# wenet-e2e/wenet

Measured on AMD Instinct MI355X. Metric: audio-seconds/sec (RTF^-1), 12L Conformer fbank80, ctc_prefix_beam_search, higher is better.
Workload: dtype f32 (feed-forward and subsampling-conv2 GEMMs: fp32 operands as three exact bf16 planes, six plane products on the bf16 matrix cores, f32 accumulate -- error <= the v_mfma_f32 kernel's, tests/test_gpu_x6.py; everything else v_mfma_f32)

## Files before the change

include/wenet_amd.h:

```cpp
#ifndef WENET_AMD_H_
#define WENET_AMD_H_

#include <stdint.h>

#ifdef __cplusplus
extern "C" {
#endif

typedef struct wn_model wn_model;

typedef struct {
  int32_t feat_dim;
  int32_t d_model;
  int32_t n_heads;
  int32_t ffn_dim;
  int32_t n_layers;
  int32_t cnn_kernel;
  int32_t causal;
  int32_t use_dynamic_chunk;
  int32_t static_chunk_size;
  int32_t vocab;
  int32_t has_cmvn;
  int32_t dec_heads;
  int32_t dec_ffn_dim;
// ... 193 lines not shown
int wn_op_mx_quantize(const float* x_dev, int32_t rows, int32_t K, void* q_dev,
                      void* scale_dev, void* stream);
int wn_op_ffn_fused(const float* X_dev, const float* W1_dev, const float* b1_dev,
                    const float* W2_dev, const float* b2_dev, float* x_inout_dev,
                    const float* ln_w_dev, const float* ln_b_dev, float* y_out_dev,
                    int32_t M, int32_t D, int32_t F, int32_t act, float alpha, float eps,
                    void* stream);
int wn_op_gemm_x6(const float* A_dev, const float* W_dev, const float* bias_dev,
                  const float* resid_dev, float* C_dev, int32_t M, int32_t N, int32_t K,
                  float alpha, int32_t act, int32_t bm, int32_t reps, void* stream);
int wn_op_ffn_x6(const float* X_dev, const float* W1_dev, const float* b1_dev,
                 const float* W2_dev, const float* b2_dev, float* x_inout_dev,
                 const float* ln_w_dev, const float* ln_b_dev, float* y_out_dev, int32_t M,
                 int32_t D, int32_t F, int32_t act, float alpha, float eps, int32_t reps,
                 void* stream);
int wn_op_gemm_x6r(const float* A_dev, const float* W_dev, const float* bias_dev,
                   float* x_inout_dev, const float* ln_w_dev, const float* ln_b_dev,
                   float* y_dev, float* C_dev, int32_t M, int32_t N, int32_t epi, float alpha,
                   float eps, int32_t reps, void* stream);

int wn_op_gemm_x6r512(const float* A, const float* W, const float* bias, float* x_inout,
                      const float* ln_w, const float* ln_b, float* y, const float* W2,
                      const float* bias2, float* C, int32_t M, int32_t N, int32_t epi, float alpha,
                      float eps, int32_t reps, void* stream);
int wn_op_log_add(const double* a_dev, const double* b_dev, double* out_dev,
                  int32_t n, void* stream);
int wn_op_layernorm(const float* x_dev, const float* w_dev, const float* b_dev,
                    float* y_dev, int32_t M, int32_t D, float eps, void* stream);

typedef struct wn_attention_op {
// ... 196 lines not shown
```

wenet_amd/_lib.py:

```python
import ctypes
import os
from ctypes import (POINTER, Structure, c_char_p, c_double, c_float, c_int32,
                    c_int64, c_void_p)

_HERE = os.path.dirname(os.path.abspath(__file__))
LIB_PATH = os.path.join(_HERE, 'libwenet_amd.so')


class WnConfig(Structure):
    _fields_ = [(n, c_int32) for n in (
        'feat_dim', 'd_model', 'n_heads', 'ffn_dim', 'n_layers', 'cnn_kernel',
        'causal', 'use_dynamic_chunk', 'static_chunk_size', 'vocab',
        'has_cmvn', 'dec_heads', 'dec_ffn_dim', 'dec_layers', 'dec_r_layers',
        'bidirectional', 'sos', 'eos', 'max_pos')] + [('norm_eps', c_float)] + [
            (n, c_int32) for n in ('encoder_type', 'input_layer', 'activation',
                                   'key_bias', 'cnn_norm',
                                   'dec_activation', 'dec_key_bias', 'dec_src_key_bias',
                                   'dec_learned_pos', 'dec_max_pos')]


class WnTransducerConfig(Structure):
    _fields_ = [(n, c_int32) for n in ('pred_embed', 'pred_hidden', 'pred_layers', 'pred_out',
                                       'join_dim', 'blank')]

# ... 25 lines not shown
                ('P', c_void_p), ('ldp', c_int32), ('p_rows', c_int32),
                ('p_off', POINTER(c_int32)), ('bias_u', c_void_p), ('bias_v', c_void_p),
                ('O', c_void_p), ('ldo', c_int32),
                ('q_off', POINTER(c_int32)), ('q_len', POINTER(c_int32)),
                ('kv_off', POINTER(c_int32)), ('kv_len', POINTER(c_int32)),
                ('n_seq', c_int32), ('n_heads', c_int32), ('mask_mode', c_int32),
                ('chunk_size', c_int32), ('left_chunks', c_int32), ('scale', c_float),
                ('flags', c_int32), ('precision', c_int32), ('x6_galign', c_int32)]


EXPORTS = [
    'wn_last_error', 'wn_version', 'wn_model_create', 'wn_model_destroy', 'wn_model_clone',
    'wn_model_set_precision', 'wn_model_get_precision', 'wn_batch_size', 'wn_model_set_encode_gate', 'wn_op_gemm_bf16',
    'wn_op_gemm_bf16_stored',
    'wn_attention_beam_search', 'wn_attention_beam_search_prompt', 'wn_attention_truncated',
    'wn_op_gemm_skinny', 'wn_encode_chunk_batch', 'wn_op_gemm_lowp', 'wn_op_mx_quantize', 'wn_op_ffn_fused', 'wn_op_gemm_x6', 'wn_op_ffn_x6', 'wn_op_gemm_x6r', 'wn_op_gemm_x6r512', 'wn_profile_kernel_name', 'wn_profile_ffn_split', 'wn_profile_ffn_clocks', 'wn_profile_gemm_clocks', 'wn_filter_blank_embedding',
    'wn_workspace_create', 'wn_resample_length', 'wn_resample', 'wn_fbank', 'wn_log_mel', 'wn_encode', 'wn_encode_chunk', 'wn_set_encoder_out',
    'wn_ctc_logprobs', 'wn_set_ctc_probs', 'wn_ctc_greedy_search', 'wn_ctc_force_align',
    'wn_set_context_graph', 'wn_ctc_prefix_beam_search', 'wn_attention_rescoring', 'wn_rescore', 'wn_rescore_prefetch', 'wn_decoder_forward', 'wn_decoder_next_topk', 'wn_op_gemm',
    'wn_op_layernorm', 'wn_op_log_add', 'wn_op_attention', 'wn_op_dwconv', 'wn_op_conv1',
    'wn_op_conv2d4',
    'wn_op_ctc_rows', 'wn_debug_set', 'wn_profile_enable',
    'wn_profile_collect', 'wn_tune_set', 'wn_model_tune_set', 'wn_tune_get',
    'wn_stream_create', 'wn_stream_destroy', 'wn_stream_set_endpoint', 'wn_stream_reset',
    'wn_stream_advance', 'wn_stream_advance_encoded',
    'wn_model_create_transducer', 'wn_transducer_greedy_search', 'wn_op_lstm_step',
    'wn_op_joint_argmax', 'wn_transducer_beam_search', 'wn_op_joint_fuse_topk',
    'wn_op_rnnt_beam_step', 'wn_transducer_beam_stats',
    'wn_rnnt_stream_create', 'wn_rnnt_stream_destroy', 'wn_rnnt_stream_reset',
    'wn_rnnt_stream_advance_encoded', 'wn_rnnt_stream_state',
    'wn_transducer_score', 'wn_transducer_score_stats', 'wn_transducer_score_times',
# ... 74 lines not shown
    L.wn_attention_beam_search.argtypes = [vp, i32, i32, f32, pi32, pi32, vp]
    L.wn_attention_beam_search_prompt.argtypes = [vp, i32, i32, f32, pi32, i32, pi32, pi32, vp]
    L.wn_attention_truncated.argtypes = [vp]
    L.wn_op_gemm.argtypes = [vp, vp, vp, vp, vp, i32, i32, i32, f32, i32, vp]
    L.wn_op_gemm_skinny.argtypes = [vp, vp, vp, vp, vp, i32, i32, i32, i32, i32, i32, vp]
    L.wn_op_gemm_bf16.argtypes = L.wn_op_gemm.argtypes
    L.wn_op_gemm_bf16_stored.argtypes = [vp, vp, vp, vp, vp, i32, i32, i32, f32, i32, i32, vp]
    L.wn_op_gemm_lowp.argtypes = [vp, vp, vp, vp, vp, vp, vp, vp, i32, i32, i32, f32, i32, i32,
                                  i32, vp]
    L.wn_op_mx_quantize.argtypes = [vp, i32, i32, vp, vp, vp]
    L.wn_op_ffn_fused.argtypes = [vp, vp, vp, vp, vp, vp, vp, vp, vp, i32, i32, i32, i32, f32,
                                  f32, vp]
    L.wn_op_gemm_x6.argtypes = [vp, vp, vp, vp, vp, i32, i32, i32, f32, i32, i32, i32, vp]
    L.wn_op_ffn_x6.argtypes = [vp, vp, vp, vp, vp, vp, vp, vp, vp, i32, i32, i32, i32, f32,
                               f32, i32, vp]
    L.wn_filter_blank_embedding.argtypes = [vp, vp, pi32, pi32, vp]
    L.wn_op_gemm_x6r.argtypes = [vp, vp, vp, vp, vp, vp, vp, vp, i32, i32, i32, f32, f32, i32, vp]
    L.wn_op_gemm_x6r512.argtypes = [vp, vp, vp, vp, vp, vp, vp, vp, vp, vp, i32, i32, i32, f32, f32,
                                    i32, vp]
    L.wn_model_set_precision.argtypes = [vp, i32]
    L.wn_model_get_precision.argtypes = [vp]
    L.wn_batch_size.argtypes = [vp]
    L.wn_batch_size.restype = i32
    L.wn_model_set_encode_gate.argtypes = [vp, vp]
    L.wn_op_layernorm.argtypes = [vp, vp, vp, vp, i32, i32, f32, vp]
    L.wn_op_log_add.argtypes = [vp, vp, vp, i32, vp]
    L.wn_op_attention.argtypes = [POINTER(WnAttentionOp), pi32, vp]
    L.wn_op_dwconv.argtypes = [vp, i32, vp, vp, vp, vp, vp, i32, vp, i32, pi32, pi32, i32, i32,
                               i32, i32, i32, i32, f32, vp]
    L.wn_op_conv1.argtypes = [vp, vp, vp, vp, vp, vp, pi32, pi32, i32, i32, i32, i32, i32, i32,
# ... 87 lines not shown
```

wenet_amd/build.py:

```python
import concurrent.futures
import hashlib
import os
import shutil
import subprocess
import sys

HERE = os.path.dirname(os.path.abspath(__file__))
CSRC = os.path.join(HERE, 'csrc')
OBJ = os.path.join(HERE, '..', 'build', 'obj')
LIB = os.path.join(HERE, 'libwenet_amd.so')
SOURCES = ['gemm.hip', 'gemm_bf16.hip', 'gemm_bf16s.hip', 'gemm_bf16p.hip', 'gemm_skinny.hip', 'ffn_fused.hip', 'gemm_rowln.hip', 'gemm_x6.hip', 'ffn_x6f.hip', 'gemm_x6r.hip', 'gemm_x6r512.hip', 'attn_search.hip', 'encoder_kernels.hip', 'attention_bf16.hip', 'attention_x6.hip', 'ctc.hip', 'ctc_align.hip', 'fbank.hip',
           'logmel.hip', 'model.hip', 'conformer.hip', 'cabi_model.hip', 'cabi_encode.hip', 'cabi_ctc.hip', 'cabi_align.hip',
           'cabi_decoder.hip', 'cabi_ops.hip', 'transducer.hip', 'transducer_beam.hip',
           'cabi_transducer.hip', 'transducer_score.hip', 'cabi_transducer_score.hip',
           'transducer_stream.hip', 'cabi_transducer_stream.hip']
FLAGS = ['--offload-arch=gfx950', '-O3', '-std=c++17', '-fPIC',
         '-fno-gpu-rdc', '-Wno-unused-result']
if os.environ.get('WN_ABLATION') == '1':
    FLAGS.append('-DWN_ABLATION')
if os.environ.get('WN_EXACT') == '1':
    FLAGS.append('-DWN_EXACT_TRANSCENDENTALS')
EXTRA_FLAGS = {'ffn_x6f.hip': ['-fno-slp-vectorize'], 'gemm_x6r.hip': ['-fno-slp-vectorize'], 'gemm_x6r512.hip': ['-fno-slp-vectorize'],
               'attention_bf16.hip': ['-fno-slp-vectorize']}


def _hipcc():
    for c in (os.environ.get('HIPCC'), shutil.which('hipcc'),
              '/opt/rocm/bin/hipcc'):
        if c and os.path.exists(c):
            return c
    raise RuntimeError('hipcc not found')


def build_host_ext(force: bool = False) -> str:
    import sysconfig
    src = os.path.join(HERE, 'cext', 'nbest_lists.c')
    out = os.path.join(HERE, '_nbest_lists' + sysconfig.get_config_var('EXT_SUFFIX'))
# ... 72 lines not shown
```

wenet_amd/csrc/cabi_ops.hip:

```cpp
#include "model_state.h"
#include "x6.h"

namespace wn {
namespace {

__global__ __launch_bounds__(256) void conv1_image_unpack_kernel(
    const char* __restrict__ img, int tiles, const int* __restrict__ t1_off,
    const int* __restrict__ t1_len, int F1, int C, float* __restrict__ out) {
  const int b = blockIdx.y;
  const int n = t1_len[b] * F1 * (C / 8);
  const int ne = (F1 + 1) / 2;
  for (int i = blockIdx.x * 256 + threadIdx.x; i < n; i += gridDim.x * 256) {
    const int cg = i % (C / 8), px = i / (C / 8);
    const int fr = px / F1, pos = px - fr * F1;
    const int f1 = pos < ne ? 2 * pos : 2 * (pos - ne) + 1;
    const int row = (t1_off[b] + fr) * F1;
    const char* src = img + x3_piece(cg >> 1, tiles, row + pos, cg & 1);
    const bf16x8 p0 = *reinterpret_cast<const bf16x8*>(src);
    const bf16x8 p1 = *reinterpret_cast<const bf16x8*>(src + X3_REC);
    const bf16x8 p2 = *reinterpret_cast<const bf16x8*>(src + 2 * X3_REC);
    float* o = out + ((int64_t)row + f1) * C + cg * 8;
#pragma unroll
    for (int e = 0; e < 8; ++e) o[e] = ((float)p0[e] + (float)p1[e]) + (float)p2[e];
  }
// ... 169 lines not shown
  if (tune().x6_af32 != 0 && (int64_t)M * K * 4 < ((int64_t)1 << 31)) {
    a.A = A; a.lda = K; a.a_bytes = (int64_t)M * K * 4;
  } else {
    WN_TRY(a3.ensure(x6_bytes(M, K)));
    WN_TRY(x6_split(A, M, K, K, a3.as<char>(), s));
    a.A3 = a3.as<char>();
  }
  a.B3 = w3.as<char>(); a.M = M; a.N = N; a.K = K; a.bm = bm;
  if (bm == 120) { a.bm = 128; a.nw = 8; }
  if (bm == 129) { a.bm = 128; a.nw = 4; }
  a.bias = bias; a.resid = resid; a.ldr = N; a.alpha = alpha; a.act = act; a.C = C; a.ldc = N;
  for (int r = 0; r < (reps > 0 ? reps : 1); ++r) WN_TRY(gemm_x6(a, s));
  return 0;
}

int wn_op_ffn_x6(const float* X, const float* W1, const float* b1, const float* W2,
                 const float* b2, float* x, const float* ln_w, const float* ln_b, float* y,
                 int32_t M, int32_t D, int32_t F, int32_t act, float alpha, float eps,
                 int32_t reps, void* stream) {
  WN_CHECK(X && W1 && b1 && W2 && b2 && x && ln_w && ln_b && y, "ffn_x6: null argument");
  WN_CHECK(M > 0 && (D == 256 || D == 512) && F > 0 && F % 64 == 0, "ffn_x6: shape");
  hipStream_t s = (hipStream_t)stream;
  static thread_local DevBuf x3, w13, w23, h3, part;
  if (tune().ffn_x6f != 0 && tune().x6_af32 == 0 && ffn_x6f_supported(M, D, F, act)) {
    FfnX6Args a;
    a.S = ffn_x6f_split(M, F);
    WN_TRY(w13.ensure(x6_bytes(F, D)));
    WN_TRY(w23.ensure(x6_bytes(D, F)));
    WN_TRY(part.ensure((size_t)a.S * M * D * sizeof(float)));
    WN_TRY(x6_split(W1, F, D, D, w13.as<char>(), s));
    WN_TRY(x6_split_perm(W2, D, F, F, w23.as<char>(), s));
    a.X = X; a.ldx = D; a.W13 = w13.as<char>(); a.W2p = w23.as<char>(); a.b1 = b1;
    a.P = part.as<float>(); a.M = M; a.D = D; a.F = F; a.act = act;
    if (tune().ffn_ximg == 2) {
      WN_TRY(x3.ensure(x6_bytes(M, D)));
      WN_TRY(x6_split(X, M, D, D, x3.as<char>(), s));
      a.X3 = x3.as<char>(); a.X = nullptr;
    }
    for (int r = 0; r < (reps > 0 ? reps : 1); ++r) WN_TRY(ffn_x6f(a, s));
    return ffn_reduce_ln(x, part.as<float>(), a.S, b2, alpha, ln_w, ln_b, nullptr, nullptr, y, M,
                         D, eps, 0, s);
  }
  const int S = ffn_x6_split(M, F);
  WN_TRY(x3.ensure(x6_bytes(M, D)));
  WN_TRY(w13.ensure(x6_bytes(F, D)));
  WN_TRY(w23.ensure(x6_bytes(D, F)));
// ... 488 lines not shown
```

wenet_amd/csrc/conformer.hip:

```cpp
#include <algorithm>
#include "model_state.h"

namespace {
struct ProfBracket {
  wn_model* m;
  hipStream_t s;
  bool on = false;
  int record(int which) { WN_HIP(hipEventRecord(m->prof_ev[m->prof_used + which], s)); return 0; }
  int begin() {
    on = m->prof_on && (m->prof_seq++ % m->prof_stride) == 0;
    if (!on) return 0;
    if (m->prof_used + 2 > m->prof_ev.size())
      for (int i = 0; i < 64; ++i) {
        hipEvent_t e;
        WN_HIP(hipEventCreate(&e));
        m->prof_ev.push_back(e);
      }
    return record(0);
  }
  int end(double flops, const char* kernel) {
    if (!on) return 0;
    WN_TRY(record(1));
    m->prof_used += 2;
    m->prof_flops += flops;
// ... 97 lines not shown
  const int d = m->cfg.d_model, M = m->rows, F = w1.out;
  const bool ximg = m->t1_img_ok;
  m->t1_img_ok = false;
  const int route = ffn_x6_route(m, w1, w2, act);
  WN_CHECK(route != 0 || !ximg,
           "ffn_x6_try: LN(x) was left as a plane image but no six-product form takes it");
  if (route == 0) return 0;
  auto i1 = W.x6_at.find(w1.w), i2 = W.x6_at.find(w2.w);
  ProfBracket pb{m, s};
  if (route == 1) {
    FfnX6Args a;
    a.S = ffn_x6f_split(M, F);
    if (m->ffn_part.ensure((size_t)a.S * M * d * sizeof(float)) != 0) return -1;
    a.X = m->t1.as<float>(); a.ldx = d; a.W13 = i1->second; a.W2p = W.x6p_at.find(w2.w)->second;
    a.b1 = w1.b;
    if (ximg) { a.X3 = m->t1_img.p; a.X = nullptr; }
    a.P = m->ffn_part.as<float>(); a.M = M; a.D = d; a.F = F; a.act = act;
    WN_TRY(pb.begin());
    if (ffn_x6f(a, s) != 0) return -1;
    WN_TRY(pb.end(4.0 * M * (double)F * d,
                  "ffn_x6f_kernel (FFN w_1 + act + w_2, six bf16 plane products)"));
    m->prof_split = a.S;
    return a.S;
  }
  const int S = ffn_x6_split(M, F);
  if (m->ffn_part.ensure((size_t)S * M * d * sizeof(float)) != 0) return -1;
  const bool af32 = tune().x6_af32 != 0 && (int64_t)M * F * 4 < ((int64_t)1 << 31);
  X6Args g1;
  g1.B3 = i1->second; g1.M = M; g1.N = F; g1.K = d; g1.bias = w1.b; g1.act = act;
  if (af32) {
// ... 431 lines not shown
```

wenet_amd/csrc/ffn_x6f.hip:

```cpp
#include <type_traits>

#include "common.h"
#include "gemm_epilogue.h"
#include "kernels.h"
#include "x6.h"

namespace wn {

namespace {

__device__ unsigned long long g_x6f_clk[4][24];

constexpr int REC = X3_REC;
constexpr int XSTAGE = 24 * REC;
constexpr int XD = 256;
constexpr int XKB = XD / 16;

typedef unsigned u32x4 __attribute__((ext_vector_type(4)));
struct Frag6 { bf16x8 p[2][3]; };

__global__ __launch_bounds__(256) void x6_split_perm_kernel(const float* __restrict__ src, int R,
                                                            int K, int ld,
                                                            char* __restrict__ dst) {
  const int tiles = (R + 31) >> 5, nkb = K >> 4;
// ... 480 lines not shown
  const int pairmap = a.S >= 2 && a.S <= 8;
  const int grid = pairmap      ? cdiv(tiles_m, 16 / a.S) * 16
                   : a.S <= 8 ? cdiv(tiles_m, 8 / a.S) * 8
                              : tiles_m * a.S;
  auto kern = ffn_x6f_kernel<ACT, RING, VAR>;
  WN_MAX_DYN_LDS(kern, 160 * 1024);
  hipLaunchKernelGGL(kern, dim3(grid), dim3(256), lds, s, a, tiles_m, pairmap);
  WN_HIP(hipGetLastError());
  return 0;
}

}


int ffn_x6f_clocks(unsigned long long* out) {
  WN_HIP(hipMemcpyFromSymbol(out, HIP_SYMBOL(g_x6f_clk), sizeof(g_x6f_clk)));
  return 0;
}

int x6_split_perm(const float* src, int R, int K, int ld, void* dst, hipStream_t s) {
  WN_CHECK(src && dst && R > 0 && K > 0 && K % 16 == 0 && ld % 4 == 0, "x6_split_perm: shape");
  const int64_t n = (int64_t)cdiv(R, 32) * (K / 16) * 64;
  hipLaunchKernelGGL(x6_split_perm_kernel, dim3((unsigned)((n + 255) / 256)), dim3(256), 0, s,
                     src, R, K, ld, reinterpret_cast<char*>(dst));
  WN_HIP(hipGetLastError());
  return 0;
}

int ffn_x6f_split(int M, int F) {
  const int tiles_m = cdiv(M, 128);
// ... 3 lines not shown
}

bool ffn_x6f_supported(int M, int D, int F, int act) {
  if (D != XD || M <= 0 || F <= 0 || F % 64 != 0) return false;
  if (act != ACT_SILU && act != ACT_RELU) return false;
  const int S = ffn_x6f_split(M, F);
  if (F % (S * 64) != 0 || F / S > 2048) return false;
  if ((int64_t)cdiv(M, 32) * X3_TILE * XKB >= ((int64_t)1 << 40)) return false;
  return tune().ffn_x6f != 3 || cdiv(M, 128) * S >= 128;
}

int ffn_x6f(const FfnX6Args& a, hipStream_t s) {
  WN_CHECK((a.X3 || (a.X && a.ldx % 4 == 0)) && a.W13 && a.W2p && a.b1 && a.P && a.M > 0 && a.D == XD && a.S > 0 &&
               a.F % (a.S * 64) == 0 && a.F / a.S <= 2048 && (a.S & (a.S - 1)) == 0 && a.S <= 32,
           "ffn_x6f: bad arguments");
#define WN_X6F(RING, VAR)                                            \
  switch (a.act) {                                                   \
    case ACT_SILU: return launch_x6f<ACT_SILU, RING, VAR>(a, s);     \
    case ACT_RELU: return launch_x6f<ACT_RELU, RING, VAR>(a, s);     \
    default: break;                                                  \
  }
  if (tune().ffn_x6f_var == 25088 && a.act == ACT_SILU) {
    if (a.X3) return launch_x6f<ACT_SILU, 3, 25088 + 32768>(a, s);
    return launch_x6f<ACT_SILU, 3, 25088>(a, s);
  }
#ifdef WN_ABLATION
  if (tune().ffn_x6f_var != 0 && a.act == ACT_SILU) {
    switch (tune().ffn_x6f_var) {
      case 1: return launch_x6f<ACT_SILU, 6, 1>(a, s);
      case 2: return launch_x6f<ACT_SILU, 6, 2>(a, s);
// ... 38 lines not shown
```

wenet_amd/csrc/kernels.h:

```cpp
#pragma once
#include "common.h"

namespace wn {

int layernorm(const float* x, int ldx, const float* w, const float* b, float* y,
              int ldy, int M, int D, float eps, hipStream_t s, bool y_bf16 = false);

int layernorm_mx(const float* x, int ldx, const float* w, const float* b, void* q,
                 unsigned* scale, int pitch, int M, int D, float eps, hipStream_t s);

int layernorm2(const float* x, const float* w1, const float* b1, const float* w2,
               const float* b2, float* y1, float* y2, int M, int D, float eps,
               hipStream_t s, bool y2_bf16 = false);

struct Conv1Args {
  const float* feats;
  const float* mean;
  const float* istd;
  const float* w;
  const float* bias;
  float* out;
  char* out3 = nullptr;
  int tiles = 0;
  const int* t1_off;
// ... 124 lines not shown
  X6CONV_256_REM128 = 2,
  X6CONV_256_KTAIL = 3
};
struct X6ConvForm {
  int tile = X6CONV_128;
  int full = 0;
  int slices = 0;
};
X6ConvForm gemm_x6_conv_form(const X6Args& a);
struct FfnX6Args {
  const float* X = nullptr;
  int ldx = 0;
  const void* X3 = nullptr;
  const void* W13 = nullptr;
  const void* W2p = nullptr;
  const float* b1 = nullptr;
  float* P = nullptr;
  int M = 0, D = 0, F = 0, S = 0, act = 0;
};
int ffn_x6f_clocks(unsigned long long* out);
int x6_split_perm(const float* src, int R, int K, int ld, void* dst, hipStream_t s);
int ffn_x6f_split(int M, int F);
bool ffn_x6f_supported(int M, int D, int F, int act);
int ffn_x6f(const FfnX6Args& a, hipStream_t s);


struct RowLnArgs {
  const float* A; int lda;
  const float* W;
  const float* bias;
  const float* resid; int ldr;
  float alpha;
  float* x_out; int ldx;
  const float* ln_w; const float* ln_b; float eps;
  float* y; int ldy;
  int M, N, K;
};
struct X6RArgs {
  const float* A = nullptr; int lda = 0;
// ... 323 lines not shown
```

wenet_amd/csrc/model.hip:

```cpp
#include <algorithm>
#include "model_state.h"

namespace wn {

static thread_local std::string g_error;
void set_error(const std::string& msg) { g_error = msg; }
const char* last_error_cstr() { return g_error.c_str(); }

}

thread_local const std::map<const float*, ModelData::MxW>* t_mx = nullptr;
thread_local const std::map<const float*, const void*>* t_x6 = nullptr;
thread_local DevBuf* t_x6_a = nullptr;

namespace wn {
Tune g_tune_default;
thread_local const Tune* t_tune = nullptr;

int* tune_field(Tune& t, const std::string& key) {
#define X(name, dflt) if (key == #name) return &t.name;
  WN_TUNE_KEYS(X)
#undef X
  return nullptr;
}

int tune_check(const std::string& key, int32_t value, const char* who) {
  if (value == TUNE_INHERIT) return 0;
  if (key == "rnnt_lookahead" && (value < 1 || value > 16)) {
    set_error(std::string(who) + ": rnnt_lookahead must be in [1, 16]");
    return -1;
  }
#ifndef WN_ABLATION
  if (key == "x6_probe" && (value & ~12) != 0) {
    set_error(std::string(who) + ": x6_probe 1 / 2 (no MFMAs / no DMA) need a WN_ABLATION build");
    return -1;
  }
  if (key == "ffn_x6f_var" && value != 0 && value != 25088) {
    set_error(std::string(who) + ": ffn_x6f_var variants other than the clock-stamp form "
              "(25088) need a WN_ABLATION build");
    return -1;
  }
  if (key == "attn_x6_var" && value != 0) {
    set_error(std::string(who) + ": attn_x6_var needs a WN_ABLATION build");
    return -1;
// ... 107 lines not shown
    char* p = W.weights_x6.as<char>();
    for (const Linear* l : ws) {
      if (!l->w || l->in % 16 != 0 || W.x6_at.count(l->w)) continue;
      WN_TRY(x6_split(l->w, l->out, l->in, l->in, p, nullptr));
      W.x6_at[l->w] = p;
      p += x6_bytes(l->out, l->in);
    }
  }
  if (cfg.d_model == 256) {
    std::vector<const Linear*> w2s;
    for (const auto& L : W.layers) { w2s.push_back(&L.ffm2); w2s.push_back(&L.ff2); }
    size_t pbytes = 0;
    for (const Linear* l : w2s)
      if (l->w && l->in % 64 == 0 && l->out == 256) pbytes += x6_bytes(l->out, l->in);
    if (pbytes > 0) {
      WN_TRY(W.weights_x6p.ensure(pbytes));
      char* q = W.weights_x6p.as<char>();
      for (const Linear* l : w2s) {
        if (!l->w || l->in % 64 != 0 || l->out != 256 || W.x6p_at.count(l->w)) continue;
        WN_TRY(x6_split_perm(l->w, l->out, l->in, l->in, q, nullptr));
        W.x6p_at[l->w] = q;
        q += x6_bytes(l->out, l->in);
      }
    }
  }
  if (cfg.d_model == 256 && cfg.n_heads == 4) {
    size_t n_q = 0;
    for (const auto& L : W.layers)
      if (L.qkv.w && L.qkv.b && L.qkv.out == 768 && L.qkv.in == 256 && L.pos_tab) ++n_q;
    if (n_q > 0) {
      const size_t img = x6_bytes(768, 256), per = img + 768 * sizeof(float);
      DevBuf stage;
      WN_TRY(stage.ensure((size_t)768 * 256 * sizeof(float)));
      WN_TRY(W.weights_x6q.ensure(n_q * per));
      char* q = W.weights_x6q.as<char>();
      for (const auto& L : W.layers) {
// ... 533 lines not shown
```

wenet_amd/csrc/model_state.h:

```cpp
#pragma once
#include <math.h>
#include <stdio.h>
#include <stdlib.h>
#include <string.h>

#include <atomic>
#include <chrono>
#include <map>
#include <memory>
#include <mutex>
#include <string>
#include <vector>

#include "../../include/wenet_amd.h"
#include "kernels.h"

namespace wn {

const char* last_error_cstr();


struct DevBuf {
  void* p = nullptr;
  size_t cap = 0;
// ... 137 lines not shown
  Linear out;
  std::vector<DecLayer> layers;
};
}

using namespace wn;


struct ModelData {
  DevBuf weights;
  int64_t n_weight_elems = 0;
  DevBuf weights_x6;
  std::map<const float*, const void*> x6_at;
  DevBuf weights_x6p;
  std::map<const float*, const void*> x6p_at;
  DevBuf weights_x6q;
  std::map<const float*, std::pair<const void*, const float*>> x6q_at;
  DevBuf bias4_buf;
  std::map<const float*, const float*> bias4;
  std::map<std::string, const float*> w;
  const float* conv1_w = nullptr; const float* conv1_b = nullptr;
  Linear conv2, sub_out;
  const float* cmvn_mean = nullptr; const float* cmvn_istd = nullptr;
  const float* pe = nullptr;
  Norm after_norm;
  Linear ctc;
  std::vector<EncLayer> layers;
  std::vector<TfLayer> tf_layers;
  Linear tconv1, tconv2;
  bool fbank_ok = true;
// ... 228 lines not shown
```

wenet_amd/csrc/tune.h:

```cpp
#pragma once
#include <stdint.h>

#include <string>

namespace wn {

#define WN_TUNE_KEYS(X)                                                                         \
                          \
  X(gemm_tile_bf16, 0)                                                                          \
                            \
  X(bf16_store, 1)                                                                              \
                      \
  X(lp_probe, 0)                                                                                \
                       \
  X(attn_split, 0)                                                                              \
                     \
  X(attn_bf16, 1)                                                                               \
                 \
  X(attn_bf16_nw, 0)                                                                            \
                                                                            \
  X(attn_bf16_defer, 80)                                                                        \
                                                              \
  X(attn_bf16_dma, 1)                                                                           \
                        \
// ... 8 lines not shown
  X(x6_linear, 1)                                                                               \
                      \
  X(x6_af32, 0)                                                                                 \
            \
  X(x6_conv_af32, 0)                                                                            \
     \
  X(enc_gate_pos, 0)                                                                            \
                                                            \
  X(x6_conv_bm, 128)                                                                            \
                    \
  X(x6_probe, 0)                                                                                \
                     \
  X(ffn_x6f, 1)                                                                                 \
            \
  X(ffn_ximg, 1)                                                                                \
                             \
  X(ffn_x6f_ring, 3)                                                                            \
                  \
  X(ffn_x6f_var, 0)                                                                             \
                                                                        \
  X(x6r, 1)                                                                                     \
                  \
  X(x6r_chain, 1)                                                                               \
          \
  X(x6r_dwc, 1)                                                                                 \
        \
  X(x6r_pro, 1)                                                                                 \
            \
  X(x6r512_rows, 0)                                                                             \
                 \
// ... 51 lines not shown
```

Measured before the change: 71310.

## Add fused FFN kernel using 16x16x32 bf16 MFMA with permuted W2 image

Adds a new fused feed-forward x6 kernel built on the 16x16x32 bf16 MFMA instruction instead of the previous 32x32 shape. It needs a W2 weight image in a new permuted layout, which is precomputed at model load alongside the existing one. A tune key selects the new kernel and defaults to it. The aim is better MFMA throughput and scheduling for the FFN GEMM chain. In exchange it doubles the permuted-weight memory and adds a large hand-scheduled kernel with its own prefetch ring and barriers.

```diff
diff --git a/include/wenet_amd.h b/include/wenet_amd.h
--- a/include/wenet_amd.h
+++ b/include/wenet_amd.h
@@ -231,6 +231,9 @@
                  const float* ln_w_dev, const float* ln_b_dev, float* y_out_dev, int32_t M,
                  int32_t D, int32_t F, int32_t act, float alpha, float eps, int32_t reps,
                  void* stream);
+int wn_op_ffn_x6_partials(const float* X_dev, const float* W1_dev, const float* b1_dev,
+                          const float* W2_dev, float* P_dev, int64_t p_floats, int32_t M,
+                          int32_t D, int32_t F, int32_t act, int32_t* S_out, void* stream);
 int wn_op_gemm_x6r(const float* A_dev, const float* W_dev, const float* bias_dev,
                    float* x_inout_dev, const float* ln_w_dev, const float* ln_b_dev,
                    float* y_dev, float* C_dev, int32_t M, int32_t N, int32_t epi, float alpha,
diff --git a/wenet_amd/_lib.py b/wenet_amd/_lib.py
--- a/wenet_amd/_lib.py
+++ b/wenet_amd/_lib.py
@@ -63,7 +63,7 @@
     'wn_model_set_precision', 'wn_model_get_precision', 'wn_batch_size', 'wn_model_set_encode_gate', 'wn_op_gemm_bf16',
     'wn_op_gemm_bf16_stored',
     'wn_attention_beam_search', 'wn_attention_beam_search_prompt', 'wn_attention_truncated',
-    'wn_op_gemm_skinny', 'wn_encode_chunk_batch', 'wn_op_gemm_lowp', 'wn_op_mx_quantize', 'wn_op_ffn_fused', 'wn_op_gemm_x6', 'wn_op_ffn_x6', 'wn_op_gemm_x6r', 'wn_op_gemm_x6r512', 'wn_profile_kernel_name', 'wn_profile_ffn_split', 'wn_profile_ffn_clocks', 'wn_profile_gemm_clocks', 'wn_filter_blank_embedding',
+    'wn_op_gemm_skinny', 'wn_encode_chunk_batch', 'wn_op_gemm_lowp', 'wn_op_mx_quantize', 'wn_op_ffn_fused', 'wn_op_gemm_x6', 'wn_op_ffn_x6', 'wn_op_ffn_x6_partials', 'wn_op_gemm_x6r', 'wn_op_gemm_x6r512', 'wn_profile_kernel_name', 'wn_profile_ffn_split', 'wn_profile_ffn_clocks', 'wn_profile_gemm_clocks', 'wn_filter_blank_embedding',
     'wn_workspace_create', 'wn_resample_length', 'wn_resample', 'wn_fbank', 'wn_log_mel', 'wn_encode', 'wn_encode_chunk', 'wn_set_encoder_out',
     'wn_ctc_logprobs', 'wn_set_ctc_probs', 'wn_ctc_greedy_search', 'wn_ctc_force_align',
     'wn_set_context_graph', 'wn_ctc_prefix_beam_search', 'wn_attention_rescoring', 'wn_rescore', 'wn_rescore_prefetch', 'wn_decoder_forward', 'wn_decoder_next_topk', 'wn_op_gemm',
@@ -168,6 +168,8 @@
     L.wn_op_gemm_x6.argtypes = [vp, vp, vp, vp, vp, i32, i32, i32, f32, i32, i32, i32, vp]
     L.wn_op_ffn_x6.argtypes = [vp, vp, vp, vp, vp, vp, vp, vp, vp, i32, i32, i32, i32, f32,
                                f32, i32, vp]
+    L.wn_op_ffn_x6_partials.argtypes = [vp, vp, vp, vp, vp, i64, i32, i32, i32, i32,
+                                        pi32, vp]
     L.wn_filter_blank_embedding.argtypes = [vp, vp, pi32, pi32, vp]
     L.wn_op_gemm_x6r.argtypes = [vp, vp, vp, vp, vp, vp, vp, vp, i32, i32, i32, f32, f32, i32, vp]
     L.wn_op_gemm_x6r512.argtypes = [vp, vp, vp, vp, vp, vp, vp, vp, vp, vp, i32, i32, i32, f32, f32,
diff --git a/wenet_amd/build.py b/wenet_amd/build.py
--- a/wenet_amd/build.py
+++ b/wenet_amd/build.py
@@ -9,7 +9,7 @@
 CSRC = os.path.join(HERE, 'csrc')
 OBJ = os.path.join(HERE, '..', 'build', 'obj')
 LIB = os.path.join(HERE, 'libwenet_amd.so')
-SOURCES = ['gemm.hip', 'gemm_bf16.hip', 'gemm_bf16s.hip', 'gemm_bf16p.hip', 'gemm_skinny.hip', 'ffn_fused.hip', 'gemm_rowln.hip', 'gemm_x6.hip', 'ffn_x6f.hip', 'gemm_x6r.hip', 'gemm_x6r512.hip', 'attn_search.hip', 'encoder_kernels.hip', 'attention_bf16.hip', 'attention_x6.hip', 'ctc.hip', 'ctc_align.hip', 'fbank.hip',
+SOURCES = ['gemm.hip', 'gemm_bf16.hip', 'gemm_bf16s.hip', 'gemm_bf16p.hip', 'gemm_skinny.hip', 'ffn_fused.hip', 'gemm_rowln.hip', 'gemm_x6.hip', 'ffn_x6f.hip', 'ffn_x6f16.hip', 'gemm_x6r.hip', 'gemm_x6r512.hip', 'attn_search.hip', 'encoder_kernels.hip', 'attention_bf16.hip', 'attention_x6.hip', 'ctc.hip', 'ctc_align.hip', 'fbank.hip',
            'logmel.hip', 'model.hip', 'conformer.hip', 'cabi_model.hip', 'cabi_encode.hip', 'cabi_ctc.hip', 'cabi_align.hip',
            'cabi_decoder.hip', 'cabi_ops.hip', 'transducer.hip', 'transducer_beam.hip',
            'cabi_transducer.hip', 'transducer_score.hip', 'cabi_transducer_score.hip',
@@ -20,7 +20,9 @@
     FLAGS.append('-DWN_ABLATION')
 if os.environ.get('WN_EXACT') == '1':
     FLAGS.append('-DWN_EXACT_TRANSCENDENTALS')
-EXTRA_FLAGS = {'ffn_x6f.hip': ['-fno-slp-vectorize'], 'gemm_x6r.hip': ['-fno-slp-vectorize'], 'gemm_x6r512.hip': ['-fno-slp-vectorize'],
+EXTRA_FLAGS = {'ffn_x6f.hip': ['-fno-slp-vectorize'],
+               'ffn_x6f16.hip': ['-fno-slp-vectorize', '-mllvm', '-pragma-unroll-threshold=131072'],
+               'gemm_x6r.hip': ['-fno-slp-vectorize'], 'gemm_x6r512.hip': ['-fno-slp-vectorize'],
                'attention_bf16.hip': ['-fno-slp-vectorize']}
 
 
diff --git a/wenet_amd/csrc/cabi_ops.hip b/wenet_amd/csrc/cabi_ops.hip
--- a/wenet_amd/csrc/cabi_ops.hip
+++ b/wenet_amd/csrc/cabi_ops.hip
@@ -207,6 +207,36 @@
   return 0;
 }
 
+int wn_op_ffn_x6_partials(const float* X, const float* W1, const float* b1, const float* W2,
+                          float* P, int64_t p_floats, int32_t M, int32_t D, int32_t F,
+                          int32_t act, int32_t* S_out, void* stream) {
+  WN_CHECK(X && W1 && b1 && W2 && P && S_out, "ffn_x6_partials: null argument");
+  WN_CHECK(M > 0 && F > 0 && ffn_x6f_supported(M, D, F, act), "ffn_x6_partials: shape");
+  hipStream_t s = (hipStream_t)stream;
+  static thread_local DevBuf x3, w13, w23;
+  FfnX6Args a;
+  a.S = ffn_x6f_split(M, F);
+  WN_CHECK((int64_t)a.S * M * D <= p_floats, "ffn_x6_partials: P is too small");
+  WN_TRY(w13.ensure(x6_bytes(F, D)));
+  WN_TRY(w23.ensure(x6_bytes(D, F)));
+  WN_TRY(x6_split(W1, F, D, D, w13.as<char>(), s));
+  if (tune().ffn_x6f_mfma == 16) {
+    WN_TRY(x6_split_perm16(W2, D, F, F, w23.as<char>(), s));
+    a.W2p16 = w23.as<char>();
+  } else {
+    WN_TRY(x6_split_perm(W2, D, F, F, w23.as<char>(), s));
+  }
+  a.X = X; a.ldx = D; a.W13 = w13.as<char>(); a.W2p = w23.as<char>(); a.b1 = b1;
+  a.P = P; a.M = M; a.D = D; a.F = F; a.act = act;
+  if (tune().ffn_ximg == 2) {
+    WN_TRY(x3.ensure(x6_bytes(M, D)));
+    WN_TRY(x6_split(X, M, D, D, x3.as<char>(), s));
+    a.X3 = x3.as<char>(); a.X = nullptr;
+  }
+  *S_out = a.S;
+  return ffn_x6f(a, s);
+}
+
 int wn_op_ffn_x6(const float* X, const float* W1, const float* b1, const float* W2,
                  const float* b2, float* x, const float* ln_w, const float* ln_b, float* y,
                  int32_t M, int32_t D, int32_t F, int32_t act, float alpha, float eps,
@@ -222,7 +252,12 @@
     WN_TRY(w23.ensure(x6_bytes(D, F)));
     WN_TRY(part.ensure((size_t)a.S * M * D * sizeof(float)));
     WN_TRY(x6_split(W1, F, D, D, w13.as<char>(), s));
-    WN_TRY(x6_split_perm(W2, D, F, F, w23.as<char>(), s));
+    if (tune().ffn_x6f_mfma == 16) {
+      WN_TRY(x6_split_perm16(W2, D, F, F, w23.as<char>(), s));
+      a.W2p16 = w23.as<char>();
+    } else {
+      WN_TRY(x6_split_perm(W2, D, F, F, w23.as<char>(), s));
+    }
     a.X = X; a.ldx = D; a.W13 = w13.as<char>(); a.W2p = w23.as<char>(); a.b1 = b1;
     a.P = part.as<float>(); a.M = M; a.D = D; a.F = F; a.act = act;
     if (tune().ffn_ximg == 2) {
diff --git a/wenet_amd/csrc/conformer.hip b/wenet_amd/csrc/conformer.hip
--- a/wenet_amd/csrc/conformer.hip
+++ b/wenet_amd/csrc/conformer.hip
@@ -135,6 +135,8 @@
     if (m->ffn_part.ensure((size_t)a.S * M * d * sizeof(float)) != 0) return -1;
     a.X = m->t1.as<float>(); a.ldx = d; a.W13 = i1->second; a.W2p = W.x6p_at.find(w2.w)->second;
     a.b1 = w1.b;
+    auto i16 = W.x6p16_at.find(w2.w);
+    if (i16 != W.x6p16_at.end()) a.W2p16 = i16->second;
     if (ximg) { a.X3 = m->t1_img.p; a.X = nullptr; }
     a.P = m->ffn_part.as<float>(); a.M = M; a.D = d; a.F = F; a.act = act;
     WN_TRY(pb.begin());
diff --git a/wenet_amd/csrc/ffn_x6f.hip b/wenet_amd/csrc/ffn_x6f.hip
--- a/wenet_amd/csrc/ffn_x6f.hip
+++ b/wenet_amd/csrc/ffn_x6f.hip
@@ -518,6 +518,7 @@
 
 
 int ffn_x6f_clocks(unsigned long long* out) {
+  if (tune().ffn_x6f_mfma == 16) return ffn_x6f16_clocks(out);
   WN_HIP(hipMemcpyFromSymbol(out, HIP_SYMBOL(g_x6f_clk), sizeof(g_x6f_clk)));
   return 0;
 }
@@ -551,6 +552,7 @@
   WN_CHECK((a.X3 || (a.X && a.ldx % 4 == 0)) && a.W13 && a.W2p && a.b1 && a.P && a.M > 0 && a.D == XD && a.S > 0 &&
                a.F % (a.S * 64) == 0 && a.F / a.S <= 2048 && (a.S & (a.S - 1)) == 0 && a.S <= 32,
            "ffn_x6f: bad arguments");
+  if (tune().ffn_x6f_mfma == 16) return ffn_x6f16(a, tune().ffn_x6f_var == 25088, s);
 #define WN_X6F(RING, VAR)                                            \
   switch (a.act) {                                                   \
     case ACT_SILU: return launch_x6f<ACT_SILU, RING, VAR>(a, s);     \
diff --git a/wenet_amd/csrc/ffn_x6f16.hip b/wenet_amd/csrc/ffn_x6f16.hip
--- /dev/null
+++ b/wenet_amd/csrc/ffn_x6f16.hip
@@ -0,0 +1,463 @@
+#include <type_traits>
+
+#include "common.h"
+#include "kernels.h"
+#include "x6.h"
+
+namespace wn {
+
+namespace {
+
+__device__ unsigned long long g_x6f16_clk[4][24];
+
+constexpr int REC = X3_REC;
+constexpr int XSTAGE = 24 * REC;
+constexpr int STG = 2 * XSTAGE;
+constexpr int RING = 3;
+constexpr int SPC = 4;
+constexpr int XD = 256;
+
+typedef unsigned u32x4 __attribute__((ext_vector_type(4)));
+
+__global__ __launch_bounds__(256) void x6_split_perm16_kernel(const float* __restrict__ src, int R,
+                                                              int K, int ld,
+                                                              char* __restrict__ dst) {
+  const int tiles = (R + 31) >> 5, nkb = K >> 4;
+  const int64_t idx = (int64_t)blockIdx.x * 256 + threadIdx.x;
+  const int row_l = (int)(idx & 31), h = (int)((idx >> 5) & 1);
+  const int64_t rest = idx >> 6;
+  const int kb = (int)(rest % nkb), tile = (int)(rest / nkb);
+  if (tile >= tiles) return;
+  const int row = tile * 32 + row_l;
+  f32x4 a = {0.f, 0.f, 0.f, 0.f}, b = a;
+  if (row < R) {
+    const float* s = src + (int64_t)row * ld + (kb >> 1) * 32 + (2 * (kb & 1) + h) * 4;
+    a = *reinterpret_cast<const f32x4*>(s);
+    b = *reinterpret_cast<const f32x4*>(s + 16);
+  }
+  bf16x8 p0, p1, p2;
+#pragma unroll
+  for (int e = 0; e < 4; ++e) {
+    const Split3 sa = split3(a[e]), sb = split3(b[e]);
+    p0[e] = sa.h0; p1[e] = sa.h1; p2[e] = sa.h2;
+    p0[4 + e] = sb.h0; p1[4 + e] = sb.h1; p2[4 + e] = sb.h2;
+  }
+  char* o = dst + ((int64_t)kb * tiles + tile) * X3_TILE + h * 512 + row_l * 16;
+  *reinterpret_cast<bf16x8*>(o) = p0;
+  *reinterpret_cast<bf16x8*>(o + REC) = p1;
+  *reinterpret_cast<bf16x8*>(o + 2 * REC) = p2;
+}
+
+template <int N>
+__device__ __forceinline__ void wait_vm() {
+  if constexpr (N == 0) asm volatile("s_waitcnt vmcnt(0)" ::: "memory");
+  else asm volatile("s_waitcnt vmcnt(12)" ::: "memory");
+}
+
+template <int ACT, bool XI, bool CLK>
+__global__ __launch_bounds__(256, 1) void ffn_x6f16_kernel(FfnX6Args p, int tiles_m, int pairmap) {
+  extern __shared__ __attribute__((aligned(16))) char smem_g[];
+  typedef __attribute__((address_space(3))) void* lds_ptr;
+  float* b1s = reinterpret_cast<float*>(smem_g + RING * STG);
+
+  const int bid = blockIdx.x, xcd = bid & 7, rr = bid >> 3;
+  int slice, tm;
+  if (pairmap && p.S >= 2 && p.S <= 8) {
+    const int nsp = p.S >> 1, pair = xcd % nsp, tg = xcd / nsp;
+    slice = 2 * pair + (rr & 1);
+    tm = (rr >> 1) * (8 / nsp) + tg;
+  } else if (p.S <= 8) {
+    slice = xcd & (p.S - 1);
+    tm = rr * (8 / p.S) + xcd / p.S;
+  } else {
+    const int sub = p.S >> 3;
+    slice = xcd + 8 * (rr % sub);
+    tm = rr / sub;
+  }
+  if (tm >= tiles_m) return;
+
+  unsigned long long clk[20] = {0, 0, 0, 0, 0, 0, 0, 0, 0, 0, 0, 0, 0, 0, 0, 0, 0, 0, 0, 0};
+  if constexpr (CLK) {
+    clk[9] = __builtin_readcyclecounter();
+    clk[12] = __builtin_amdgcn_s_memrealtime();
+  }
+  const int tid = threadIdx.x, lane = tid & 63;
+  const int wave = __builtin_amdgcn_readfirstlane(tid >> 6);
+  __builtin_assume(wave >= 0 && wave < 4);
+  const int gq = lane >> 4, li = lane & 15;
+  const int NC = p.F / p.S / 64;
+  const int cg0 = slice * NC;
+  const int FT = p.F >> 5;
+  const unsigned vlane = (unsigned)lane * 16u;
+  const int offA = (gq >> 1) * 3 * REC + (gq & 1) * 512 + li * 16;
+  const int offB = (gq >> 1) * XSTAGE + (gq & 1) * 512 + li * 16;
+
+  const __amdgpu_buffer_rsrc_t r1 = __builtin_amdgcn_make_buffer_rsrc(
+      const_cast<char*>(reinterpret_cast<const char*>(p.W13)), 0,
+      (int)((int64_t)p.F * XD * 6), 0x00020000);
+  const __amdgpu_buffer_rsrc_t r2 = __builtin_amdgcn_make_buffer_rsrc(
+      const_cast<char*>(reinterpret_cast<const char*>(p.W2p16)), 0,
+      (int)((int64_t)p.F * XD * 6), 0x00020000);
+
+  auto issue_one = [&](int c, int sub, int buf, int j) {
+    char* dst = smem_g + buf * STG + (sub & 1) * XSTAGE + wave * 6 * REC + j * REC;
+    const int cg = cg0 + c;
+    if (sub < 4) {
+      const int nt = sub >> 1, j2 = j / 3, pl = j - j2 * 3;
+      const int ks = (sub & 1) * 8 + wave * 2 + j2;
+      const int so = ((ks * FT + 2 * cg + nt) * 3) * REC;
+      __builtin_amdgcn_raw_ptr_buffer_load_lds(r1, (lds_ptr)dst, 16, vlane, so + pl * REC, 0, 0);
+    } else {
+      const int so = ((cg * 4 + sub - 4) * 24 + wave * 6) * REC;
+      __builtin_amdgcn_raw_ptr_buffer_load_lds(r2, (lds_ptr)dst, 16, vlane, so + j * REC, 0, 0);
+    }
+  };
+  auto issue = [&](int c, int st, int buf) {
+#pragma unroll
+    for (int h = 0; h < 2; ++h)
+#pragma unroll
+      for (int j = 0; j < 6; ++j) issue_one(c, st * 2 + h, buf, j);
+  };
+
+  bf16x8 X[8][2][3];
+  f32x4 xa[8][2], xb[8][2];
+  f32x4 xr[4][8];
+  if constexpr (XI) {
+    const int tiles = (p.M + 31) >> 5;
+    const int tile = min(tm * 4 + wave, tiles - 1);
+    const char* xi = reinterpret_cast<const char*>(p.X3) + (int64_t)tile * X3_TILE +
+                     (gq & 1) * 512 + li * 16;
+    const int64_t kstr = (int64_t)tiles * X3_TILE;
+#pragma unroll
+    for (int kb2 = 0; kb2 < 8; ++kb2)
+#pragma unroll
+      for (int r = 0; r < 2; ++r)
+#pragma unroll
+        for (int pl = 0; pl < 3; ++pl)
+          X[kb2][r][pl] = *reinterpret_cast<const bf16x8*>(xi + (2 * kb2 + (gq >> 1)) * kstr +
+                                                           pl * REC + r * 256);
+  } else {
+    const int r4 = lane >> 4, c16 = lane & 15;
+#pragma unroll
+    for (int q = 0; q < 4; ++q)
+#pragma unroll
+      for (int j = 0; j < 8; ++j) {
+        const int row = min(tm * 128 + wave * 32 + 4 * j + r4, p.M - 1);
+        xr[q][j] = *reinterpret_cast<const f32x4*>(p.X + (int64_t)row * p.ldx + q * 64 + c16 * 4);
+      }
+  }
+#pragma unroll
+  for (int t = 0; t < RING - 1; ++t) issue(0, t, t);
+  float b1v[8];
+#pragma unroll
+  for (int i = 0; i < 8; ++i) b1v[i] = p.b1[cg0 * 64 + min(tid + 256 * i, NC * 64 - 1)];
+  if constexpr (CLK) { __builtin_amdgcn_sched_barrier(0); clk[15] = __builtin_readcyclecounter(); __builtin_amdgcn_sched_barrier(0); }
+  if constexpr (!XI) {
+    char* patch = smem_g + (RING - 1) * STG + wave * (32 * 272);
+    const int r4 = lane >> 4, c16 = lane & 15;
+#pragma unroll
+    for (int q = 0; q < 4; ++q) {
+#pragma unroll
+      for (int j = 0; j < 8; ++j)
+        *reinterpret_cast<f32x4*>(patch + (4 * j + r4) * 272 + c16 * 16) = xr[q][j];
+#pragma unroll
+      for (int k2 = 0; k2 < 2; ++k2)
+#pragma unroll
+        for (int r = 0; r < 2; ++r) {
+          const char* s = patch + (16 * r + li) * 272 + k2 * 128 + gq * 32;
+          xa[2 * q + k2][r] = *reinterpret_cast<const f32x4*>(s);
+          xb[2 * q + k2][r] = *reinterpret_cast<const f32x4*>(s + 16);
+        }
+      asm volatile("s_waitcnt lgkmcnt(0)" ::: "memory");
+    }
+#pragma unroll
+    for (int kb2 = 0; kb2 < 8; ++kb2)
+#pragma unroll
+      for (int r = 0; r < 2; ++r)
+#pragma unroll
+        for (int e = 0; e < 4; ++e) {
+          const Split3 sa = split3(xa[kb2][r][e]), sb = split3(xb[kb2][r][e]);
+          X[kb2][r][0][e] = sa.h0; X[kb2][r][1][e] = sa.h1; X[kb2][r][2][e] = sa.h2;
+          X[kb2][r][0][4 + e] = sb.h0; X[kb2][r][1][4 + e] = sb.h1; X[kb2][r][2][4 + e] = sb.h2;
+        }
+  }
+  if constexpr (CLK) { __builtin_amdgcn_sched_barrier(0); clk[16] = __builtin_readcyclecounter(); __builtin_amdgcn_sched_barrier(0); }
+  asm volatile("s_waitcnt vmcnt(0)" ::: "memory");
+  if constexpr (CLK) { __builtin_amdgcn_sched_barrier(0); clk[17] = __builtin_readcyclecounter(); __builtin_amdgcn_sched_barrier(0); }
+#pragma unroll
+  for (int kb2 = 0; kb2 < 8; ++kb2)
+#pragma unroll
+    for (int r = 0; r < 2; ++r)
+#pragma unroll
+      for (int pl = 0; pl < 3; ++pl) asm volatile("" : "+v"(X[kb2][r][pl]));
+#pragma unroll
+  for (int i = 0; i < 8; ++i)
+    if (tid + 256 * i < NC * 64) b1s[tid + 256 * i] = b1v[i];
+  __syncthreads();
+  if constexpr (CLK) { __builtin_amdgcn_sched_barrier(0); clk[18] = __builtin_readcyclecounter(); __builtin_amdgcn_sched_barrier(0); }
+
+  f32x4 Y[16][2];
+#pragma unroll
+  for (int t = 0; t < 16; ++t)
+#pragma unroll
+    for (int r = 0; r < 2; ++r) Y[t][r] = f32x4{0.f, 0.f, 0.f, 0.f};
+  f32x4 H[2][2][2];
+  u32x4 Hp[2][2][3];
+
+  constexpr int PW[6] = {2, 0, 1, 1, 0, 0}, PX[6] = {0, 2, 1, 0, 1, 0};
+  constexpr int RT[6] = {0, 1, 0, 1, 0, 1}, RP[6] = {2, 2, 0, 0, 1, 1};
+
+  float pv0 = 0.f, pv1 = 0.f, pt0 = 0.f, pt1 = 0.f;
+  unsigned ph0 = 0, ph1 = 0;
+  auto pk = [](float a, float b) {
+    typedef __bf16 bf16x2 __attribute__((ext_vector_type(2)));
+    const bf16x2 h = {(__bf16)a, (__bf16)b};
+    return __builtin_bit_cast(unsigned, h);
+  };
+  auto lo = [](unsigned u) { return __builtin_bit_cast(float, u << 16); };
+  auto hi16 = [](unsigned u) { return __builtin_bit_cast(float, u & 0xffff0000u); };
+  auto piece_slice = [&](int nt, int pi, int k, const f32x4& bq) {
+    const int u = pi >> 2, r = (pi >> 1) & 1, q0 = 2 * (pi & 1);
+    switch (k) {
+      case 0: {
+        float b0 = bq[q0];
+        asm volatile("" : "+v"(b0));
+        pv0 = H[nt][u][r][q0] + b0;
+        break;
+      }
+      case 1: {
+        float b1 = bq[q0 + 1];
+        asm volatile("" : "+v"(b1));
+        pv1 = H[nt][u][r][q0 + 1] + b1;
+        break;
+      }
+      case 2:
+        if (ACT == ACT_SILU) { asm volatile("" : "+v"(pv0)); pt0 = pv0 * -1.4426950408889634f; }
+        break;
+      case 3:
+        if (ACT == ACT_SILU) { asm volatile("" : "+v"(pv1)); pt1 = pv1 * -1.4426950408889634f; }
+        break;
+      case 4:
+        if (ACT == ACT_SILU) { asm volatile("" : "+v"(pt0)); pt0 = wn_exp2(pt0); }
+        break;
+      case 5:
+        if (ACT == ACT_SILU) { asm volatile("" : "+v"(pt1)); pt1 = wn_exp2(pt1); }
+        break;
+      case 6:
+        if (ACT == ACT_SILU) { asm volatile("" : "+v"(pt0)); pt0 = 1.0f + pt0; }
+        break;
+      case 7:
+        if (ACT == ACT_SILU) { asm volatile("" : "+v"(pt1)); pt1 = 1.0f + pt1; }
+        break;
+      case 8:
+        if (ACT == ACT_SILU) { asm volatile("" : "+v"(pt0)); pt0 = wn_rcp(pt0); }
+        break;
+      case 9:
+        if (ACT == ACT_SILU) { asm volatile("" : "+v"(pt1)); pt1 = wn_rcp(pt1); }
+        break;
+      case 10:
+        asm volatile("" : "+v"(pv0));
+        if (ACT == ACT_SILU) { asm volatile("" : "+v"(pt0)); pv0 *= pt0; }
+        if (ACT == ACT_RELU) pv0 = fmaxf(pv0, 0.0f);
+        break;
+      case 11:
+        asm volatile("" : "+v"(pv1));
+        if (ACT == ACT_SILU) { asm volatile("" : "+v"(pt1)); pv1 *= pt1; }
+        if (ACT == ACT_RELU) pv1 = fmaxf(pv1, 0.0f);
+        break;
+      case 12:
+        asm volatile("" : "+v"(pv0), "+v"(pv1));
+        ph0 = pk(pv0, pv1);
+        break;
+      case 13:
+        asm volatile("" : "+v"(pv0), "+v"(ph0));
+        pv0 -= lo(ph0);
+        break;
+      case 14:
+        asm volatile("" : "+v"(pv1), "+v"(ph0));
+        pv1 -= hi16(ph0);
+        break;
+      case 15:
+        asm volatile("" : "+v"(pv0), "+v"(pv1));
+        ph1 = pk(pv0, pv1);
+        break;
+      case 16:
+        asm volatile("" : "+v"(pv0), "+v"(ph1));
+        pv0 -= lo(ph1);
+        break;
+      case 17:
+        asm volatile("" : "+v"(pv1), "+v"(ph1));
+        pv1 -= hi16(ph1);
+        break;
+      case 18: {
+        asm volatile("" : "+v"(pv0), "+v"(pv1));
+        const int d = 2 * u + (q0 >> 1);
+        Hp[nt][r][0][d] = ph0;
+        Hp[nt][r][1][d] = ph1;
+        Hp[nt][r][2][d] = pk(pv0, pv1);
+        break;
+      }
+      default: break;
+    }
+  };
+  auto read_frag = [&](bool phase_a, int b, int gs, int u, int pl) {
+    const int o = phase_a ? (gs * 6 + pl) * REC + offA : (gs * 3 + pl) * REC + offB;
+    return *reinterpret_cast<const bf16x8*>(smem_g + b * STG + o + u * 256);
+  };
+  const f32x4 zero4 = {0.f, 0.f, 0.f, 0.f};
+
+  int buf = 0;
+  bf16x8 fc[2][3];
+#pragma unroll
+  for (int q = 0; q < 6; ++q) fc[RT[q]][RP[q]] = read_frag(true, 0, 0, RT[q], RP[q]);
+  if constexpr (CLK) clk[10] = __builtin_readcyclecounter();
+  auto chunk = [&](auto last_tag, int c) {
+    constexpr bool last = decltype(last_tag)::value;
+    f32x4 bq = {0.f, 0.f, 0.f, 0.f};
+#pragma unroll
+    for (int st = 0; st < SPC; ++st) {
+#pragma unroll
+      for (int gs = 0; gs < 8; ++gs) {
+        if constexpr (CLK && !last) {
+          if ((gs & 3) == 0) {
+            __builtin_amdgcn_sched_barrier(0);
+            clk[2 * st + (gs >> 2)] = __builtin_readcyclecounter();
+            __builtin_amdgcn_sched_barrier(0);
+          }
+        }
+        bf16x8 fn[2][3];
+        const bool do_piece = st == 1 || st == 2;
+        const int pnt = st == 2 ? 1 : 0;
+        const int pi = gs;
+        if (do_piece && (pi & 3) == 0)
+          bq = *reinterpret_cast<const f32x4*>(b1s + c * 64 + pnt * 32 + 16 * (pi >> 2) + 4 * gq);
+#pragma unroll
+        for (int k = 0; k < 24; ++k) {
+          const int q = k >> 2, u = (k >> 1) & 1, r = k & 1;
+          if (st < 2) {
+            const bool first = gs == 0 && q == 0;
+            H[st][u][r] = __builtin_amdgcn_mfma_f32_16x16x32_bf16(
+                fc[u][PW[q]], X[gs][r][PX[q]], first ? zero4 : H[st][u][r], 0, 0, 0);
+          } else {
+            const bf16x8 hb = __builtin_bit_cast(bf16x8, Hp[st - 2][r][PX[q]]);
+            Y[2 * gs + u][r] = __builtin_amdgcn_mfma_f32_16x16x32_bf16(fc[u][PW[q]], hb,
+                                                                       Y[2 * gs + u][r], 0, 0, 0);
+          }
+          if (gs == 7 && k == 11) {
+            __builtin_amdgcn_sched_barrier(0);
+            asm volatile("s_waitcnt lgkmcnt(0)" ::: "memory");
+            if (last && st >= SPC - 2) wait_vm<0>(); else wait_vm<12>();
+            __builtin_amdgcn_s_barrier();
+            buf = buf + 1 == RING ? 0 : buf + 1;
+            __builtin_amdgcn_sched_barrier(0);
+          }
+          {
+            const int ka = do_piece ? 21 : 5, kb = do_piece ? 22 : 17;
+            if ((k == ka || k == kb) && gs < 6) {
+              const int j12 = gs * 2 + (k == kb ? 1 : 0);
+              const int tst = st + RING - 1;
+              const int bufp = buf == 0 ? RING - 1 : buf - 1;
+              if (tst < SPC) issue_one(c, tst * 2 + j12 / 6, bufp, j12 % 6);
+              else if (!last) issue_one(c + 1, (tst - SPC) * 2 + j12 / 6, bufp, j12 % 6);
+            }
+          }
+          if (gs < 7) {
+            if ((k & 3) == 3) fn[RT[q]][RP[q]] = read_frag(st < 2, buf, gs + 1, RT[q], RP[q]);
+          } else if (k >= 12 && (k & 1) == 0 && (st < SPC - 1 || !last)) {
+            const int i6 = (k - 12) >> 1;
+            fn[RT[i6]][RP[i6]] = read_frag(st == 0 || st == SPC - 1, buf, 0, RT[i6], RP[i6]);
+          }
+          if (do_piece) piece_slice(pnt, pi, k, bq);
+          __builtin_amdgcn_sched_barrier(0);
+        }
+        if (gs < 7 || st < SPC - 1 || !last) {
+#pragma unroll
+          for (int u = 0; u < 2; ++u)
+#pragma unroll
+            for (int pl = 0; pl < 3; ++pl) fc[u][pl] = fn[u][pl];
+        }
+      }
+    }
+    if constexpr (CLK && !last) clk[8] = __builtin_readcyclecounter();
+  };
+  for (int c = 0; c + 1 < NC; ++c) chunk(std::false_type{}, c);
+  chunk(std::true_type{}, NC - 1);
+
+  if constexpr (CLK) clk[11] = __builtin_readcyclecounter();
+  __syncthreads();
+  char* patch = smem_g + wave * (32 * 1040);
+#pragma unroll
+  for (int t = 0; t < 16; ++t)
+#pragma unroll
+    for (int r = 0; r < 2; ++r)
+      *reinterpret_cast<f32x4*>(patch + (16 * r + li) * 1040 + (16 * t + 4 * gq) * 4) = Y[t][r];
+  float* P0 = p.P + ((int64_t)slice * p.M + tm * 128 + wave * 32) * XD + lane * 4;
+  const int nrow = min(32, p.M - (tm * 128 + wave * 32));
+#pragma unroll
+  for (int r = 0; r < 32; ++r) {
+    const f32x4 v = *reinterpret_cast<const f32x4*>(patch + r * 1040 + lane * 16);
+    if (r < nrow) *reinterpret_cast<f32x4*>(P0 + (int64_t)r * XD) = v;
+  }
+  if constexpr (CLK) {
+    asm volatile("s_waitcnt vmcnt(0)" ::: "memory");
+    clk[13] = __builtin_amdgcn_s_memrealtime();
+    const unsigned long long t_end = __builtin_readcyclecounter();
+    if (blockIdx.x == gridDim.x / 2 && lane == 0) {
+#pragma unroll
+      for (int i = 0; i < 20; ++i) g_x6f16_clk[wave][i] = clk[i];
+      g_x6f16_clk[wave][20] = t_end;
+    }
+  }
+}
+
+template <int ACT, bool XI, bool CLK>
+int launch_x6f16(const FfnX6Args& a, hipStream_t s) {
+  const int tiles_m = cdiv(a.M, 128);
+  const int NC = a.F / a.S / 64;
+  const size_t lds = (size_t)RING * STG + (size_t)NC * 64 * sizeof(float);
+  const int pairmap = a.S >= 2 && a.S <= 8;
+  const int grid = pairmap      ? cdiv(tiles_m, 16 / a.S) * 16
+                   : a.S <= 8 ? cdiv(tiles_m, 8 / a.S) * 8
+                              : tiles_m * a.S;
+  auto kern = ffn_x6f16_kernel<ACT, XI, CLK>;
+  WN_MAX_DYN_LDS(kern, 160 * 1024);
+  hipLaunchKernelGGL(kern, dim3(grid), dim3(256), lds, s, a, tiles_m, pairmap);
+  WN_HIP(hipGetLastError());
+  return 0;
+}
+
+}
+
+int ffn_x6f16_clocks(unsigned long long* out) {
+  WN_HIP(hipMemcpyFromSymbol(out, HIP_SYMBOL(g_x6f16_clk), sizeof(g_x6f16_clk)));
+  return 0;
+}
+
+int x6_split_perm16(const float* src, int R, int K, int ld, void* dst, hipStream_t s) {
+  WN_CHECK(src && dst && R > 0 && K > 0 && K % 32 == 0 && ld % 4 == 0, "x6_split_perm16: shape");
+  const int64_t n = (int64_t)cdiv(R, 32) * (K / 16) * 64;
+  hipLaunchKernelGGL(x6_split_perm16_kernel, dim3((unsigned)((n + 255) / 256)), dim3(256), 0, s,
+                     src, R, K, ld, reinterpret_cast<char*>(dst));
+  WN_HIP(hipGetLastError());
+  return 0;
+}
+
+int ffn_x6f16(const FfnX6Args& a, bool clocks, hipStream_t s) {
+  WN_CHECK(a.W2p16, "ffn_x6f16: no 16x16x32 image of W2 (x6_split_perm16)");
+  if (clocks && a.act == ACT_SILU)
+    return a.X3 ? launch_x6f16<ACT_SILU, true, true>(a, s)
+                : launch_x6f16<ACT_SILU, false, true>(a, s);
+  switch (a.act) {
+    case ACT_SILU:
+      return a.X3 ? launch_x6f16<ACT_SILU, true, false>(a, s)
+                  : launch_x6f16<ACT_SILU, false, false>(a, s);
+    case ACT_RELU:
+      return a.X3 ? launch_x6f16<ACT_RELU, true, false>(a, s)
+                  : launch_x6f16<ACT_RELU, false, false>(a, s);
+    default: break;
+  }
+  set_error("ffn_x6f16: unsupported activation");
+  return -1;
+}
+
+}
diff --git a/wenet_amd/csrc/kernels.h b/wenet_amd/csrc/kernels.h
--- a/wenet_amd/csrc/kernels.h
+++ b/wenet_amd/csrc/kernels.h
@@ -162,6 +162,7 @@
   const void* X3 = nullptr;
   const void* W13 = nullptr;
   const void* W2p = nullptr;
+  const void* W2p16 = nullptr;
   const float* b1 = nullptr;
   float* P = nullptr;
   int M = 0, D = 0, F = 0, S = 0, act = 0;
@@ -171,6 +172,9 @@
 int ffn_x6f_split(int M, int F);
 bool ffn_x6f_supported(int M, int D, int F, int act);
 int ffn_x6f(const FfnX6Args& a, hipStream_t s);
+int x6_split_perm16(const float* src, int R, int K, int ld, void* dst, hipStream_t s);
+int ffn_x6f16(const FfnX6Args& a, bool clocks, hipStream_t s);
+int ffn_x6f16_clocks(unsigned long long* out);
 
 
 struct RowLnArgs {
diff --git a/wenet_amd/csrc/model.hip b/wenet_amd/csrc/model.hip
--- a/wenet_amd/csrc/model.hip
+++ b/wenet_amd/csrc/model.hip
@@ -28,6 +28,10 @@
   if (value == TUNE_INHERIT) return 0;
   if (key == "rnnt_lookahead" && (value < 1 || value > 16)) {
     set_error(std::string(who) + ": rnnt_lookahead must be in [1, 16]");
+    return -1;
+  }
+  if (key == "ffn_x6f_mfma" && value != 32 && value != 16) {
+    set_error(std::string(who) + ": ffn_x6f_mfma must be 32 or 16");
     return -1;
   }
 #ifndef WN_ABLATION
@@ -165,12 +169,15 @@
     for (const Linear* l : w2s)
       if (l->w && l->in % 64 == 0 && l->out == 256) pbytes += x6_bytes(l->out, l->in);
     if (pbytes > 0) {
-      WN_TRY(W.weights_x6p.ensure(pbytes));
+      WN_TRY(W.weights_x6p.ensure(2 * pbytes));
       char* q = W.weights_x6p.as<char>();
       for (const Linear* l : w2s) {
         if (!l->w || l->in % 64 != 0 || l->out != 256 || W.x6p_at.count(l->w)) continue;
         WN_TRY(x6_split_perm(l->w, l->out, l->in, l->in, q, nullptr));
         W.x6p_at[l->w] = q;
+        q += x6_bytes(l->out, l->in);
+        WN_TRY(x6_split_perm16(l->w, l->out, l->in, l->in, q, nullptr));
+        W.x6p16_at[l->w] = q;
         q += x6_bytes(l->out, l->in);
       }
     }
diff --git a/wenet_amd/csrc/model_state.h b/wenet_amd/csrc/model_state.h
--- a/wenet_amd/csrc/model_state.h
+++ b/wenet_amd/csrc/model_state.h
@@ -175,6 +175,7 @@
   std::map<const float*, const void*> x6_at;
   DevBuf weights_x6p;
   std::map<const float*, const void*> x6p_at;
+  std::map<const float*, const void*> x6p16_at;
   DevBuf weights_x6q;
   std::map<const float*, std::pair<const void*, const float*>> x6q_at;
   DevBuf bias4_buf;
diff --git a/wenet_amd/csrc/tune.h b/wenet_amd/csrc/tune.h
--- a/wenet_amd/csrc/tune.h
+++ b/wenet_amd/csrc/tune.h
@@ -46,6 +46,8 @@
   X(ffn_x6f, 1)                                                                                 \
             \
   X(ffn_ximg, 1)                                                                                \
+                    \
+  X(ffn_x6f_mfma, 16)                                                                           \
                              \
   X(ffn_x6f_ring, 3)                                                                            \
                   \
```

Result: faster. 72530 (median of 6 runs) (+1.7%).
